# ndjinga/CirculantPreconditioner

Measured on AMD Instinct MI355X. Metric: PCApply/s on 256^3 complex grid, higher is better.
Workload: dtype c128 (f64 complex); 1 GPU; 256x256x256 c128 circulant PCApply, transport symbol lambda=(0.6, 0.15, 0.02); global_batch=1, parallelism=single GPU

## Files before the change

circulantpreconditioner_amd/csrc/cfp_three_pass.hip:

```cpp
#include "cfp_fft_device.h"
#include "cfp_lane.h"
#include "cfp_three_pass.h"

#include <hip/hip_ext.h>

#ifndef CFP_REAL_MID_XCD
#define CFP_REAL_MID_XCD 1
#endif

#define TP_LAUNCH(K, G, B, S, ...)                                                                    \
  do {                                                                                                \
    if (g_stamp.start || g_stamp.stop)                                                                \
      hipExtLaunchKernelGGL(K, G, B, 0, S, g_stamp.start, g_stamp.stop, 0, __VA_ARGS__);              \
    else                                                                                              \
      hipLaunchKernelGGL(K, G, B, 0, S, __VA_ARGS__);                                                 \
  } while (0)

namespace cfp {

namespace {

__device__ __forceinline__ cd dft4_dif(cd v, int q) {
  const cd p = dpp_c<DPP_XOR2>(v);
  cd t = (q & 2) ? csub(p, v) : cadd(v, p);
// ... 411 lines not shown
    }
    {
      const Col q = column(u);
#pragma unroll
      for (int m = 0; m < PTS; ++m)
        if constexpr (!(PROBE & PR_NO_Y2)) v[m] = dft4_dit(v[m], q.y2 & 3);
#pragma unroll
      for (int m = 0; m < PTS; ++m) {
        if constexpr ((PROBE & PR_NO_Y2) != 0) {
          v[m] = cmul(v[m], q.w);
          continue;
        }
        if constexpr (N2 >= 8) {
          const cd u = (q.y2 & 4) ? cmul(v[m], q.w8) : v[m];
          const cd p = lane_xor4(u);
          v[m] = (q.y2 & 4) ? csub(p, u) : cadd(u, p);
        }
        if constexpr (N2 == 16) {
          const cd u = (q.y2 & 8) ? cmul(v[m], q.w16) : v[m];
          const cd p = lane_xor8(u);
          v[m] = (q.y2 & 8) ? csub(p, u) : cadd(u, p);
        }
        v[m] = cmul(v[m], q.w);
      }
      if constexpr (PROBE & PR_NO_STORE) {
        double acc = 0.0;
#pragma unroll
        for (int m = 0; m < PTS; ++m) acc += v[m].x + v[m].y;
        if (acc == 1.2345e300) q.col[0] = make_cd(acc, 0.0);
      } else {
#pragma unroll
        for (int m = 0; m < PTS; ++m) gstore<FLAGS>(q.col + zs * TZ * m, cconj(v[m]));
      }
    }
    lds_barrier();
  }
}

namespace {
__device__ __forceinline__ double ror8_d(double v) {
  const long long b = __double_as_longlong(v);
  const int lo = __builtin_amdgcn_mov_dpp((int)(b & 0xffffffffll), 0x128, 0xf, 0xf, false);
  const int hi = __builtin_amdgcn_mov_dpp((int)(b >> 32), 0x128, 0xf, 0xf, false);
  return __longlong_as_double(((long long)hi << 32) | (unsigned int)lo);
}
__device__ __forceinline__ cd bfly_l3(cd v, double sgn) {
  return make_cd(fma(sgn, v.x, ror8_d(v.x)), fma(sgn, v.y, ror8_d(v.y)));
}
}

template <int B, int D, bool TW = true, int NR = 16>
__device__ __forceinline__ void dif_pairs(cd* v, cd w) {
#pragma unroll
  for (int k = 0; k < NR; ++k)
    if ((k & D) == 0) swap_c<B>(v[k], v[k + D]);
#pragma unroll
  for (int k = 0; k < NR; ++k)
    if ((k & D) == 0) {
      const cd a = v[k], b = v[k + D];
      v[k] = cadd(a, b);
      v[k + D] = TW ? cmul(csub(a, b), w) : csub(a, b);
    }
}

typedef __attribute__((address_space(3))) void lds_void_t;
typedef __attribute__((address_space(1))) void glb_void_t;
template <int T, int N2, int TN, int PROBE = 0, bool PF = false, int NX = TN, int ST = 0, int LD = 0, bool BL = false,
          bool XCD = false, int TAG = 0>
__global__ void __launch_bounds__(T * (TN / 16)) __attribute__((amdgpu_waves_per_eu(4)))
k_tp_mid_sw(cd* data, TPArgs a, int nunits) {
#ifndef CFP_KEXP
  static_assert(PROBE == 0, "timing probes are built in tools/kexp only");
#endif
  static_assert(T == 64 || (T == 32 && N2 == 8), "a wave = the 64 columns of one z group, or 32 columns of two");
  static_assert(N2 == 4 || N2 == 8, "y2 = the top 2 or 3 lane bits");
  static_assert(TN == 256, "z = 16 x 16: radix-16 stage A in registers, one exchange, radix-16 stage B");
  constexpr int N1 = TN / N2, TZ = TN / 16, NT = T * TZ, XT = T / N2, NXT = NX / XT;
  constexpr int XB = ilog2(XT);
  static_assert(NX % XT == 0, "whole x tiles");
  static_assert(!BL || (NX == TN && N2 == 8), "blocked layout: complex grid, 8 x times 8 y2");
  __shared__ __attribute__((aligned(16))) double lds[T * TN];
  __shared__ cd tw_l[TN];
  const int tid = threadIdx.x;
  for (int i = tid; i < TN; i += NT) tw_l[i] = a.tw[i];
  __syncthreads();
  const int lane0 = tid & 63;
  const int c0 = T == 64 ? lane0 : (lane0 & 3) | ((lane0 >> 3) << 2);
  const int tz0 = T == 64 ? tid / 64 : 2 * (tid >> 6) + ((lane0 >> 2) & 1);
  const i64 zs = (i64)NX << (a.lnyl ? a.lnyl : ilog2(TN));
  const auto idx = [](int i) {
    asm volatile("" : "+v"(i));
    return i;
  };
  const auto col_ptr = [&](int u, int c, int tz) {
    const int xt = u % NXT, k1 = u / NXT;
    if constexpr (BL) return data + (i64)NX * N2 * k1 + xt * T + c + zs * tz;
    return data + xt * XT + (c & (XT - 1)) + (i64)NX * ((c >> XB) + N2 * k1) + zs * tz;
  };
  const auto tw_y = [&](int u, int c) { return tw_l[((c >> XB) * (a.k1_off + u / NXT)) & (TN - 1)]; };
  constexpr int NPF = PF ? 8 : 0;
  const int wv = __builtin_amdgcn_readfirstlane(tid / 64);
  if constexpr ((PROBE & PR_PRIO) != 0) {
    if (wv >= NT / 128) __builtin_amdgcn_s_setprio(1);
  }
  const auto prefetch = [&](int u) {
    const int c = idx(c0), tz = idx(tz0);
    const cd* src = col_ptr(u, c, tz);
#pragma unroll
    for (int m = 0; m < NPF; ++m)
      __builtin_amdgcn_global_load_lds((glb_void_t*)(src + zs * TZ * m), (lds_void_t*)(lds + (wv * NPF + m) * 128),
                                       16, 0, (LD & F_NT_LD) ? 2 : 0);
  };
  static_assert(!PF || (NT / 64) * NPF * 128 <= T * TN, "the prefetch fits the exchange buffer");
  if constexpr (PF) {
    if ((int)blockIdx.x < nunits) prefetch(XCD ? xcd_unit(blockIdx.x, gridDim.x) : (int)blockIdx.x);
  }
  const auto exchange_t = [&](cd* v, bool first) {
    if constexpr (PROBE & PR_NO_XCHG) return;
    const int c = idx(c0), tz = idx(tz0), lane = idx(lane0);
    const int l3 = N2 == 8 ? ((lane >> 3) & 1) : 0, l4 = (lane >> 4) & 1, l5 = (lane >> 5) & 1;
    const int wbase = (tz * 16 + l5 + 2 * l4) * T + (c & (XT - 1)) + XT * l3;
#pragma unroll
    for (int h = 0; h < 2; ++h) {
      if (!(first && h == 0)) lds_barrier();
#pragma unroll
      for (int r = 0; r < 16; ++r) {
        const int p = N2 == 8 ? 4 * (r & 1) + 2 * ((r >> 1) & 1) : 2 * (r & 1) + ((r >> 1) & 1);
        const int off = (r & 12) * T + XT * (N2 == 8 ? p & 6 : p);
        lds[wbase + off] = h ? v[r].y : v[r].x;
      }
      lds_barrier();
#pragma unroll
      for (int t = 0; t < 16; ++t) {
        const double d = lds[(tz + TZ * t) * T + c];
        if (h) v[t].y = d; else v[t].x = d;
      }
    }
  };
  const auto stage_b = [&](cd* v) {
    if constexpr (PROBE & PR_NO_ZMATH) return;
    const int tz = idx(tz0);
#pragma unroll
    for (int t = 1; t < 16; ++t) v[t] = cmul(v[t], tw_l[tz * t]);
    dft_reg<16>(v);
  };
  const auto lane_sign = [&]() {
    const int lane = idx(lane0);
    return (lane & 8) ? -1.0 : 1.0;
  };

  for (int it = blockIdx.x; it < nunits; it += gridDim.x) {
    const int u = XCD ? xcd_unit(it, gridDim.x) : it;
    cd v[16];
    if constexpr (PROBE & PR_NO_LOAD) {
      const int c = idx(c0), tz = idx(tz0);
#pragma unroll
      for (int m = 0; m < 16; ++m) v[m] = make_cd(c + m, tz + u);
    } else {
      const int c = idx(c0), tz = idx(tz0);
      const cd* src = col_ptr(u, c, tz);
#pragma unroll
      for (int m = NPF; m < 16; ++m) v[m] = gload<LD>(src + zs * TZ * m);
      if constexpr (PF) {
        asm volatile("s_waitcnt vmcnt(0)" ::: "memory");
#pragma unroll
        for (int m = 0; m < NPF; ++m) {
          const int lane = idx(lane0);
          v[m] = fromv(*reinterpret_cast<const dv2*>(lds + (wv * NPF + m) * 128 + 2 * lane));
        }
      }
    }
    {
      const int c = idx(c0);
      const cd w = tw_y(u, c);
#pragma unroll
      for (int m = 0; m < 16; ++m) v[m] = cmul(v[m], w);
    }
    if constexpr (!(PROBE & PR_NO_ZMATH)) dft_reg<16>(v);
    if constexpr (PROBE & PR_NO_Y2) {
    } else if constexpr (N2 == 8) {
      {
        const int lane = idx(lane0);
        dif_pairs<5, 1>(v, tw_l[(TN / 8) * ((lane >> 3) & 3)]);
      }
      {
        const int lane = idx(lane0);
        dif_pairs<4, 2>(v, tw_l[(TN / 4) * ((lane >> 3) & 1)]);
      }
      const double s = lane_sign();
#pragma unroll
      for (int r = 0; r < 16; ++r) v[r] = bfly_l3(v[r], s);
    } else {
      {
        const int lane = idx(lane0);
        dif_pairs<5, 1>(v, tw_l[(TN / 4) * ((lane >> 4) & 1)]);
      }
      dif_pairs<4, 2, false>(v, make_cd(1.0, 0.0));
    }
    exchange_t(v, !PF);
    stage_b(v);
    {
      const int c = idx(c0), tz = idx(tz0);
      const int k1 = a.k1_off + u / NXT, p = c >> XB;
      const cd cs = a.colsym[(u % NXT) * XT + (c & (XT - 1)) + (i64)NX * (k1 + N1 * brev<N2>(p))];
#pragma unroll
      for (int m = 0; m < 16; ++m) {
        const cd d = cadd(cadd(cs, a.axsym[tz + TZ * m]), make_cd(1.0, 0.0));
        v[m] = (PROBE & PR_NO_ZMATH) ? cconj(v[m]) : cconj(cdiv_sym(v[m], d));
      }
    }
    if constexpr (!(PROBE & PR_NO_ZMATH)) dft_reg<16>(v);
    if constexpr (PROBE & PR_NO_Y2) {
    } else if constexpr (N2 == 8) {
      {
        const double s = lane_sign();
#pragma unroll
        for (int r = 0; r < 16; ++r) v[r] = bfly_l3(v[r], s);
      }
      {
        const int lane = idx(lane0);
        const cd w = tw_l[(TN / 4) * ((lane >> 3) & 1)];
#pragma unroll
        for (int k = 0; k < 16; ++k)
          if ((k & 2) == 0) swap_c<4>(v[k], v[k + 2]);
#pragma unroll
        for (int k = 0; k < 16; ++k)
          if ((k & 2) == 0) {
            const cd x = v[k], y = cmul(v[k + 2], w);
            v[k] = cadd(x, y);
            v[k + 2] = csub(x, y);
          }
      }
      {
        const int lane = idx(lane0);
        const cd w = tw_l[(TN / 8) * ((lane >> 3) & 1)];
#pragma unroll
        for (int k = 0; k < 16; ++k)
          if ((k & 1) == 0) swap_c<5>(v[k], v[k + 1]);
#pragma unroll
        for (int k = 0; k < 16; ++k)
          if ((k & 1) == 0) {
            cd y = cmul(v[k + 1], w);
            if (k & 2) y = mul_mi(y);
            const cd x = v[k];
            v[k] = cadd(x, y);
            v[k + 1] = csub(x, y);
          }
      }
    } else {
#pragma unroll
      for (int k = 0; k < 16; ++k)
        if ((k & 2) == 0) swap_c<4>(v[k], v[k + 2]);
#pragma unroll
      for (int k = 0; k < 16; ++k)
        if ((k & 2) == 0) {
          const cd x = v[k], y = v[k + 2];
          v[k] = cadd(x, y);
          v[k + 2] = csub(x, y);
        }
#pragma unroll
      for (int k = 0; k < 16; ++k)
        if ((k & 1) == 0) swap_c<5>(v[k], v[k + 1]);
#pragma unroll
      for (int k = 0; k < 16; ++k)
        if ((k & 1) == 0) {
          const cd y = (k & 2) ? mul_mi(v[k + 1]) : v[k + 1];
          const cd x = v[k];
          v[k] = cadd(x, y);
          v[k + 1] = csub(x, y);
        }
    }
    exchange_t(v, false);
    if constexpr (PF) {
      lds_barrier();
      if (it + (int)gridDim.x < nunits) prefetch(XCD ? xcd_unit(it + gridDim.x, gridDim.x) : it + (int)gridDim.x);
    }
    stage_b(v);
    {
      const int c = idx(c0), tz = idx(tz0);
      const cd w = tw_y(u, c);
      cd* dst = col_ptr(u, c, tz);
      if constexpr (PROBE & PR_NO_STORE) {
        double acc = 0.0;
#pragma unroll
        for (int m = 0; m < 16; ++m) acc += v[m].x * w.x + v[m].y;
        if (acc == 1.2345e300) dst[0] = make_cd(acc, 0.0);
      } else {
#pragma unroll
        for (int m = 0; m < 16; ++m) gstore<ST>(dst + zs * TZ * m, cconj(cmul(v[m], w)));
      }
    }
    if constexpr (!PF) lds_barrier();
  }
}

constexpr int kRecNPF = 7;
template <int PROBE, bool PF, int LD>
__device__ __forceinline__ void tp_mid_rec_body(cd* __restrict__ data, const TPArgs& a, int nunits,
                                                double* __restrict__ pf_l, cd* __restrict__ carr,
                                                cd* __restrict__ ctab, cd* __restrict__ tw_l) {
  constexpr int TN = 256, N2 = 8, N1 = TN / N2, XT = 8, NXT = TN / XT, NW = 16;
  constexpr int NPF = PF ? kRecNPF : 0;
  const int tid = threadIdx.x;
  const int lane = tid & 63, x = lane & 7, zl = lane >> 3;
  const int wv = __builtin_amdgcn_readfirstlane(tid / 64);
  const i64 zs = (i64)TN << (a.lnyl ? a.lnyl : ilog2(TN));
  const cd lz = a.lamz;
  const auto idx = [](int i) {
    asm volatile("" : "+v"(i));
    return i;
  };
  const auto colsym_of = [&](int u) {
    return a.colsym[(u % NXT) * XT + x + (i64)TN * (a.k1_off + u / NXT + N1 * zl)];
  };
  const auto ctab_put = [&](int buf, cd cs) {
    const cd den = make_cd(cs.x + 1.0 + lz.x, cs.y + lz.y);
    const double id = 1.0 / fma(den.x, den.x, den.y * den.y);
    const cd ri = make_cd(den.x * id, -den.y * id);
    ctab[(2 * buf) * 64 + idx(lane)] = cmul(lz, ri);
    ctab[(2 * buf + 1) * 64 + idx(lane)] = make_cd(ri.x * (double)TN, ri.y * (double)TN);
  };
  if (tid < TN) tw_l[tid] = a.tw[tid];
  if (wv == 0 && (int)blockIdx.x < nunits) ctab_put(0, colsym_of((int)blockIdx.x));
  __syncthreads();
  const unsigned loff = 16u * ((unsigned)x + (unsigned)zs * 2u * (unsigned)zl);
  const auto slot_ptr = [&](int u, int m) {
    return data + ((u % NXT) * XT + (i64)TN * (N2 * (u / NXT) + (m & 7)) + zs * (16 * wv + (m >> 3)));
  };
  const auto at = [](cd* base, unsigned off) { return reinterpret_cast<cd*>(reinterpret_cast<char*>(base) + off); };
  const auto prefetch = [&](int u) {
    unsigned lo0 = loff;
    asm volatile("" : "+s"(u), "+v"(lo0));
#pragma unroll
    for (int m = 0; m < NPF; ++m)
      __builtin_amdgcn_global_load_lds((glb_void_t*)at(slot_ptr(u, m), lo0), (lds_void_t*)(pf_l + (wv * NPF + m) * 128),
                                       16, 0, (LD & F_NT_LD) ? 2 : 0);
  };
  if constexpr (PF) {
    if ((int)blockIdx.x < nunits) prefetch((int)blockIdx.x);
  }
  const bool up3 = (zl & 1) != 0, up4 = (zl & 2) != 0, up5 = (zl & 4) != 0;
  const cd zero = make_cd(0.0, 0.0), one = make_cd(1.0, 0.0);
  const auto pin = [](cd& w) { asm volatile("" : "+v"(w.x), "+v"(w.y)); };
  const auto cfma = [](cd p, cd q, cd c) {
    return make_cd(fma(p.x, q.x, fma(-p.y, q.y, c.x)), fma(p.x, q.y, fma(p.y, q.x, c.y)));
  };

  int par = 0, buf = 0;
  const auto unit = [&](const int it, auto more_c) {
    constexpr bool more = decltype(more_c)::value;
    const int u = it;
    const int k1 = a.k1_off + u / NXT;
    const int nbuf = buf == 2 ? 0 : buf + 1;
    cd v[16], csn = zero;
    if constexpr (PROBE & PR_NO_LOAD) {
#pragma unroll
      for (int m = 0; m < 16; ++m) v[m] = make_cd(lane + m, wv + u);
    } else {
      if constexpr (PF) {
        asm volatile("s_waitcnt vmcnt(0)" ::: "memory");
#pragma unroll
        for (int m = 0; m < NPF; ++m)
          v[m] = fromv(*reinterpret_cast<const dv2*>(pf_l + (wv * NPF + m) * 128 + 2 * idx(lane)));
      }
      if constexpr (more) csn = colsym_of(it + (int)gridDim.x);
      {
        int ul = u;
        unsigned lo1 = loff;
        asm volatile("" : "+s"(ul), "+v"(lo1));
#pragma unroll
        for (int m = NPF; m < 16; ++m) v[m] = gload<LD>(at(slot_ptr(ul, m), lo1));
      }
    }
    if (more && wv == 0) ctab_put(nbuf, csn);
#pragma unroll
    for (int y = 1; y < N2; ++y) {
      const cd w = tw_l[(y * k1) & (TN - 1)];
      v[y] = cmul(v[y], w);
      v[8 + y] = cmul(v[8 + y], w);
    }
    if constexpr (PF && more && !(PROBE & PR_NO_LOAD)) {
#pragma unroll
      for (int m = 0; m < 16; ++m) pin(v[m]);
      prefetch(it + (int)gridDim.x);
    }
    __builtin_amdgcn_sched_barrier(0);
    if constexpr (!(PROBE & PR_NO_Y2)) {
      dft_reg<8>(v);
#pragma unroll
      for (int m = 0; m < 8; ++m) pin(v[m]);
      __builtin_amdgcn_sched_barrier(0);
      dft_reg<8>(v + 8);
#pragma unroll
      for (int m = 8; m < 16; ++m) pin(v[m]);
      __builtin_amdgcn_sched_barrier(0);
    }
    if constexpr (!(PROBE & PR_NO_ZMATH)) {
      const auto pow2zl = [&](cd aa) {
        cd pw = cmul(aa, aa), q = up3 ? pw : one;
        pw = cmul(pw, pw);
        q = up4 ? cmul(q, pw) : q;
        pw = cmul(pw, pw);
        return up5 ? cmul(q, pw) : q;
      };
#pragma unroll
      for (int k2 = 0; k2 < 8; ++k2) {
        const int c = (idx(lane) & 7) + 8 * k2;
        const cd aa = ctab[(2 * buf) * 64 + c], r = ctab[(2 * buf + 1) * 64 + c];
        const cd v0 = cmul(v[k2], r), v1 = cmul(v[8 + k2], r);
        cd S = cfma(aa, v0, v1), X, lo, hi, pw = cmul(aa, aa), q;
        __builtin_amdgcn_sched_barrier(0);
        {
          const cd pr = lane_xor8(S);
          lo = up3 ? pr : S;
          hi = up3 ? S : pr;
          X = up3 ? lo : zero;
          S = cfma(pw, lo, hi);
          q = up3 ? pw : one;
          pw = cmul(pw, pw);
        }
        __builtin_amdgcn_sched_barrier(0);
        {
          lo = S;
          hi = S;
          swap_c<4>(lo, hi);
          if (up4) X = cfma(q, lo, X);
          S = cfma(pw, lo, hi);
          q = up4 ? cmul(q, pw) : q;
          pw = cmul(pw, pw);
        }
        __builtin_amdgcn_sched_barrier(0);
        {
          lo = S;
          hi = S;
          swap_c<5>(lo, hi);
          if (up5) X = cfma(q, lo, X);
          S = cfma(pw, lo, hi);
        }
        v[k2] = cfma(aa, X, v0);
        v[8 + k2] = cfma(aa, v[k2], v1);
        pin(v[k2]);
        pin(v[8 + k2]);
        if (zl == k2) carr[(par * NW + wv) * 64 + idx(lane)] = S;
        __builtin_amdgcn_sched_barrier(0);
      }
      lds_barrier();
      cd cin;
      {
        const int ln = idx(lane);
        const cd am = ctab[(2 * buf) * 64 + ln];
        const cd am2 = cmul(am, am), am4 = cmul(am2, am2), am8 = cmul(am4, am4);
        const cd A = cmul(am8, am8);
        cd acc = carr[(par * NW + wv) * 64 + ln];
#pragma unroll
        for (int k = 14; k >= 0; --k) {
          acc = cfma(acc, A, carr[(par * NW + ((wv - 1 - k) & 15)) * 64 + ln]);
          if ((k & 3) == 0) __builtin_amdgcn_sched_barrier(0);
        }
        const cd A2 = cmul(A, A), A4 = cmul(A2, A2), A8 = cmul(A4, A4), A16 = cmul(A8, A8);
        const cd d = make_cd(1.0 - A16.x, -A16.y);
        const double id = 1.0 / fma(d.x, d.x, d.y * d.y);
        cin = make_cd(fma(acc.x, d.x, acc.y * d.y) * id, fma(acc.y, d.x, -acc.x * d.y) * id);
      }
#pragma unroll
      for (int k2 = 0; k2 < 8; ++k2) {
        const int c = (idx(lane) & 7) + 8 * k2;
        const long long bx = __double_as_longlong(cin.x), by = __double_as_longlong(cin.y);
        const unsigned xl = (unsigned)__builtin_amdgcn_ds_bpermute(4 * c, (int)(bx & 0xffffffffll));
        const unsigned xh = (unsigned)__builtin_amdgcn_ds_bpermute(4 * c, (int)(bx >> 32));
        const unsigned yl = (unsigned)__builtin_amdgcn_ds_bpermute(4 * c, (int)(by & 0xffffffffll));
        const unsigned yh = (unsigned)__builtin_amdgcn_ds_bpermute(4 * c, (int)(by >> 32));
        const cd ci = make_cd(__longlong_as_double((long long)(((unsigned long long)xh << 32) | xl)),
                              __longlong_as_double((long long)(((unsigned long long)yh << 32) | yl)));
        const cd aa = ctab[(2 * buf) * 64 + c];
        const cd g = cmul(cmul(aa, pow2zl(aa)), ci);
        v[k2] = cadd(v[k2], g);
        v[8 + k2] = cfma(aa, g, v[8 + k2]);
        pin(v[k2]);
        pin(v[8 + k2]);
        __builtin_amdgcn_sched_barrier(0);
      }
    }
#pragma unroll
    for (int m = 0; m < 16; ++m) v[m] = cconj(v[m]);
    if constexpr (!(PROBE & PR_NO_Y2)) {
      dft_reg<8>(v);
#pragma unroll
      for (int m = 0; m < 8; ++m) pin(v[m]);
      __builtin_amdgcn_sched_barrier(0);
      dft_reg<8>(v + 8);
#pragma unroll
      for (int m = 8; m < 16; ++m) pin(v[m]);
      __builtin_amdgcn_sched_barrier(0);
    }
    {
      int k1s = k1, us = u;
      unsigned lo2 = loff;
      asm volatile("" : "+s"(k1s), "+s"(us), "+v"(lo2));
      if constexpr (PROBE & PR_NO_STORE) {
        double acc = 0.0;
#pragma unroll
        for (int m = 0; m < 16; ++m) acc += v[m].x + v[m].y;
        if (acc == 1.2345e300) *at(slot_ptr(us, 0), lo2) = make_cd(acc, 0.0);
      } else {
#pragma unroll
        for (int m = 0; m < 16; ++m) {
          const cd w = (m & 7) ? tw_l[((m & 7) * k1s) & (TN - 1)] : one;
          gstore<0>(at(slot_ptr(us, m), lo2), cconj(cmul(v[m], w)));
        }
      }
    }
    par ^= 1;
    buf = nbuf;
  };
  int it = blockIdx.x;
  for (; it + (int)gridDim.x < nunits; it += gridDim.x) unit(it, std::true_type{});
  if (it < nunits) unit(it, std::false_type{});
}

template <int PROBE = 0, bool PF = false, int LD = 0, int TAG = 0>
__global__ void __launch_bounds__(1024) __attribute__((amdgpu_waves_per_eu(4)))
k_tp_mid_rec(cd* data, TPArgs a, int nunits) {
#ifndef CFP_KEXP
  static_assert(PROBE == 0, "timing probes are built in tools/kexp only");
#endif
  __shared__ __attribute__((aligned(16))) double pf_l[PF ? 16 * kRecNPF * 128 : 2];
  __shared__ __attribute__((aligned(16))) cd carr[2 * 16 * 64];
  __shared__ __attribute__((aligned(16))) cd ctab[3 * 2 * 64];
  __shared__ cd tw_l[256];
  tp_mid_rec_body<PROBE, PF, LD>(data, a, nunits, pf_l, carr, ctab, tw_l);
}


bool three_pass_supported(const i64 n[3]) {
  return n[0] == n[1] && n[1] == n[2] && (n[0] == 128 || n[0] == 256 || n[0] == 512);
}

static int cu_count() {
  static int cus = 0;
  if (!cus) {
    int dev = 0;
    if (hipGetDevice(&dev) != hipSuccess ||
        hipDeviceGetAttribute(&cus, hipDeviceAttributeMultiprocessorCount, dev) != hipSuccess || cus < 1)
      cus = 256;
  }
  return cus;
}

static unsigned grid_of(int units, int per_cu) {
  const int g = per_cu * cu_count();
  return (unsigned)(units < g ? units : g);
}
static unsigned grid_xcd(int units, int per_cu) {
  unsigned g = grid_of(units, per_cu), p = 1;
  while (2 * p <= g) p *= 2;
  return p >= 8 && units % p == 0 ? p : 0;
}

template <bool INV, int M = 128, int N1 = 32, int N2 = 8, int NY = 256, int MF = 0, int OCC = 4, bool WC = false,
          bool WL = false>
__global__ void __launch_bounds__(N1 * (M / 8)) __attribute__((amdgpu_waves_per_eu(OCC)))
k_tp_rows_r2c(const double* in_r, cd* H, cd* Q, double* out_r, TPArgs a, int nunits) {
  constexpr int PTS = 8;
  constexpr int TPC = M / PTS;
  constexpr int TY = N1 / PTS;
  constexpr int NT = N1 * TPC;
  constexpr int RS = M + M / 16;
  constexpr int TC = WL ? M + 16 : M;
  static_assert(!WL || (64 % TPC == 0 && TY * 16 == 64 && M % 16 == 0), "wave-local: whole rows and 16 columns per wave");
  constexpr int F = (WC ? 0 : F_SPLIT_LDS) | F_LDS_SYNC;
  constexpr int FW = F | (WL ? F_WAVE_LDS : 0);
  constexpr int LDS_D = (N1 * RS > N1 * TC ? N1 * RS : N1 * TC) * (WC ? 2 : 1);
  __shared__ __attribute__((aligned(16))) double lds[LDS_D];
  cd* const lc = reinterpret_cast<cd*>(lds);
  __shared__ cd tw_m[M];
  __shared__ cd tw_1[N1];
  __shared__ cd qy[N1];
  const int tid = threadIdx.x;
  for (int i = tid; i < M; i += NT) tw_m[i] = a.tw[2 * i];
  for (int i = tid; i < N1; i += NT) tw_1[i] = a.tw[(2 * M / N1) * i];
  if constexpr (WL) __syncthreads();
  const int r0 = tid / TPC, tpc0 = tid % TPC;
  const int x0 = WL ? (tid >> 6) * 16 + (tid & 15) : tid % M, ty0 = WL ? (tid >> 4) & 3 : tid / M;
  const auto idx = [](int i) {
    asm volatile("" : "+v"(i));
    return i;
  };
  const auto to_columns_r2c = [&](cd* v, int z, int y2) {
    const int r = idx(r0), tpc = idx(tpc0), x = idx(x0), ty = idx(ty0);
    const int xm = (M - x) & (M - 1);
    cd zm[PTS];
    if constexpr (WC) {
      lds_barrier();
#pragma unroll
      for (int t = 0; t < PTS; ++t) {
        const int k = tpc + TPC * t;
        lc[r * RS + k + (k >> 4)] = v[t];
      }
      lds_barrier();
#pragma unroll
      for (int m = 0; m < PTS; ++m) {
        const int row = (ty + TY * m) * RS;
        v[m] = lc[row + x + (x >> 4)];
        zm[m] = lc[row + xm + (xm >> 4)];
      }
    } else {
#pragma unroll
      for (int h = 0; h < 2; ++h) {
        lds_barrier();
#pragma unroll
        for (int t = 0; t < PTS; ++t) {
          const int k = tpc + TPC * t;
          lds[r * RS + k + (k >> 4)] = h ? v[t].y : v[t].x;
        }
        lds_barrier();
#pragma unroll
        for (int m = 0; m < PTS; ++m) {
          const int row = (ty + TY * m) * RS;
          const double d = lds[row + x + (x >> 4)], dm = lds[row + xm + (xm >> 4)];
          if (h) { v[m].y = d; zm[m].y = dm; } else { v[m].x = d; zm[m].x = dm; }
        }
      }
    }
    lds_barrier();
    const cd w = a.tw[x];
#pragma unroll
    for (int m = 0; m < PTS; ++m) {
      const cd e = make_cd(0.5 * (v[m].x + zm[m].x), 0.5 * (v[m].y - zm[m].y));
      const cd d = make_cd(v[m].x - zm[m].x, v[m].y + zm[m].y);
      const cd o = make_cd(0.5 * d.y, -0.5 * d.x);
      v[m] = cadd(e, cmul(w, o));
      if (x == 0) qy[ty + TY * m] = csub(e, o);
    }
  };
  const auto to_rows_c2r = [&](cd* v, int z, int y2) {
    const int r = idx(r0), tpc = idx(tpc0), x = idx(x0), ty = idx(ty0);
    cd xm[PTS];
    if constexpr (WC) {
      lds_barrier();
#pragma unroll
      for (int m = 0; m < PTS; ++m) lc[(ty + TY * m) * RS + x + (x >> 4)] = cconj(v[m]);
      lds_barrier();
#pragma unroll
      for (int t = 0; t < PTS; ++t) {
        const int k = tpc + TPC * t, km = (M - k) & (M - 1);
        v[t] = lc[r * RS + k + (k >> 4)];
        xm[t] = lc[r * RS + km + (km >> 4)];
      }
    } else {
#pragma unroll
      for (int h = 0; h < 2; ++h) {
        lds_barrier();
#pragma unroll
        for (int m = 0; m < PTS; ++m) lds[(ty + TY * m) * RS + x + (x >> 4)] = h ? -v[m].y : v[m].x;
        lds_barrier();
#pragma unroll
        for (int t = 0; t < PTS; ++t) {
          const int k = tpc + TPC * t, km = (M - k) & (M - 1);
          const double d = lds[r * RS + k + (k >> 4)], dm = lds[r * RS + km + (km >> 4)];
          if (h) { v[t].y = d; xm[t].y = dm; } else { v[t].x = d; xm[t].x = dm; }
        }
      }
    }
    lds_barrier();
    if (tpc == 0) xm[0] = qy[r];
#pragma unroll
    for (int t = 0; t < PTS; ++t) {
      const int k = tpc + TPC * t;
      const cd e = make_cd(0.5 * (v[t].x + xm[t].x), 0.5 * (v[t].y - xm[t].y));
      const cd d = make_cd(0.5 * (v[t].x - xm[t].x), 0.5 * (v[t].y + xm[t].y));
      const cd o = cmul(d, cconj(a.tw[k]));
      v[t] = cconj(make_cd(e.x - o.y, e.y + o.x));
    }
  };
  for (int u = blockIdx.x; u < nunits; u += gridDim.x) {
    const int z = u / N2, y2 = u % N2;
    cd v[PTS];
    if constexpr (!INV) {
      {
        const int r = idx(r0), tpc = idx(tpc0);
        const cd* src = reinterpret_cast<const cd*>(in_r) + ((i64)z * NY + y2 + N2 * r) * M + tpc;
#pragma unroll
        for (int t = 0; t < PTS; ++t) v[t] = gload<MF>(src + TPC * t);
        __builtin_amdgcn_sched_barrier(0);
        fft_stages<M, PTS, r0_of(M, PTS), true, N1, FW>(v, lds, tw_m, r, tpc, true);
      }
      to_columns_r2c(v, z, y2);
      {
        const int x = idx(x0), ty = idx(ty0);
        fft_stages<N1, PTS, r0_of(N1, PTS), false, TC, FW>(v, lds, tw_1, x, ty, true);
        cd* dst = H + ((i64)z * NY + y2 + N2 * ty) * M + x;
#pragma unroll
        for (int m = 0; m < PTS; ++m) dst[(i64)N2 * TY * M * m] = v[m];
      }
      if constexpr (WL) asm volatile("s_waitcnt lgkmcnt(0)" ::: "memory");
      if (tid < N1) {
        const int k = idx(tid);
        cd acc = make_cd(0.0, 0.0);
#pragma unroll 8
        for (int j = 0; j < N1; ++j) acc = cadd(acc, cmul(qy[j], tw_1[(j * k) & (N1 - 1)]));
        Q[(i64)z * NY + y2 + N2 * k] = acc;
      }
    } else {
      cd qk = make_cd(0.0, 0.0);
      if (tid < N1) qk = Q[(i64)z * NY + y2 + N2 * idx(tid)];
      {
        const int x = idx(x0), ty = idx(ty0);
        const cd* src = H + ((i64)z * NY + y2 + N2 * ty) * M + x;
#pragma unroll
        for (int m = 0; m < PTS; ++m) v[m] = src[(i64)N2 * TY * M * m];
        __builtin_amdgcn_sched_barrier(0);
#pragma unroll
        for (int m = 0; m < PTS; ++m) v[m] = cconj(v[m]);
        fft_stages<N1, PTS, r0_of(N1, PTS), false, TC, FW>(v, lds, tw_1, x, ty, true);
      }
      if (tid < 64) {
        if (tid < N1) qy[tid] = qk;
        asm volatile("s_waitcnt lgkmcnt(0)" ::: "memory");
        cd acc = make_cd(0.0, 0.0);
        const int y1 = idx(tid) & (N1 - 1);
#pragma unroll 8
        for (int k = 0; k < N1; ++k) acc = cadd(acc, cmul(qy[k], cconj(tw_1[(y1 * k) & (N1 - 1)])));
        asm volatile("s_waitcnt lgkmcnt(0)" ::: "memory");
        if (tid < N1) qy[tid] = acc;
      }
      to_rows_c2r(v, z, y2);
      {
        const int r = idx(r0), tpc = idx(tpc0);
        fft_stages<M, PTS, r0_of(M, PTS), true, N1, FW>(v, lds, tw_m, r, tpc, true);
        const double sc = a.scale;
        cd* dst = reinterpret_cast<cd*>(out_r) + ((i64)z * NY + y2 + N2 * r) * M + tpc;
#pragma unroll
        for (int t = 0; t < PTS; ++t) gstore<MF>(dst + TPC * t, make_cd(v[t].x * sc, -v[t].y * sc));
      }
    }
    lds_barrier();
  }
}

hipError_t launch_three_pass_real(int stage, int n, const double* b, cd* H, cd* Q, double* x, const TPArgs& a,
                                  hipStream_t s, bool alt_rows) {
  if (stage == 3) {
    if (n == 128)
      hipLaunchKernelGGL((k_tp_mid<0, 4, 4, 128, 8, false, 1>), dim3(32), dim3(4 * 16), 0, s, Q, a, 32);
    else
      hipLaunchKernelGGL((k_tp_mid<0, 8, 8, 256, 4, false, 1>), dim3(32), dim3(8 * 64), 0, s, Q, a, 32);
    return hipGetLastError();
  }
  if (n == 128) {
    if (stage == 1) {
      constexpr int units = (64 / 8) * 32;
      hipLaunchKernelGGL((k_tp_mid<0, 32, 4, 128, 8, false, 64>), dim3(grid_of(units, 2)), dim3(512), 0, s, H, a,
                         units);
    } else {
      constexpr int units = 128 * 4;
      const unsigned g = grid_of(units, 4);
      if (stage == 0 && alt_rows)
        hipLaunchKernelGGL((k_tp_rows_r2c<false, 64, 32, 4, 128>), dim3(g), dim3(256), 0, s, b, H, Q, nullptr, a,
                           units);
      else if (stage == 0)
        hipLaunchKernelGGL((k_tp_rows_r2c<false, 64, 32, 4, 128, 0, 4, false, true>), dim3(g), dim3(256), 0, s, b, H,
                           Q, nullptr, a, units);
      else if (alt_rows)
        hipLaunchKernelGGL((k_tp_rows_r2c<true, 64, 32, 4, 128>), dim3(g), dim3(256), 0, s, nullptr, H, Q, x, a,
                           units);
      else
        hipLaunchKernelGGL((k_tp_rows_r2c<true, 64, 32, 4, 128, 0, 4, false, true>), dim3(g), dim3(256), 0, s, nullptr,
                           H, Q, x, a, units);
    }
    return hipGetLastError();
  }
  if (stage == 1) {
    constexpr int units = (128 / 8) * 32;
    const unsigned gx = CFP_REAL_MID_XCD ? grid_xcd(units, 1) : 0;
    if (gx)
      hipLaunchKernelGGL((k_tp_mid_sw<64, 8, 256, 0, true, 128, 0, 0, false, true>), dim3(gx), dim3(1024), 0, s, H, a,
                         units);
    else
      hipLaunchKernelGGL((k_tp_mid_sw<64, 8, 256, 0, true, 128>), dim3(grid_of(units, 1)), dim3(1024), 0, s, H, a,
                         units);
  } else {
    constexpr int units = 256 * 8;
    const unsigned g = grid_of(units, 2);
    if (stage == 0 && !alt_rows)
      hipLaunchKernelGGL((k_tp_rows_r2c<false, 128, 32, 8, 256, F_NT_LD, 6, false, true>), dim3(grid_of(units, 3)),
                         dim3(512), 0, s, b, H, Q, nullptr, a, units);
    else if (stage == 0)
      hipLaunchKernelGGL((k_tp_rows_r2c<false, 128, 32, 8, 256, F_NT_LD, 6>), dim3(grid_of(units, 3)), dim3(512), 0, s, b,
                         H, Q, nullptr, a, units);
    else if (!alt_rows)
      hipLaunchKernelGGL((k_tp_rows_r2c<true, 128, 32, 8, 256, F_NT_ST, 4, true, true>), dim3(g), dim3(512), 0, s,
                         nullptr, H, Q, x, a, units);
    else
      hipLaunchKernelGGL((k_tp_rows_r2c<true, 128, 32, 8, 256, F_NT_ST, 4, true>), dim3(g), dim3(512), 0, s, nullptr, H, Q, x, a,
                         units);
  }
  return hipGetLastError();
}


constexpr int kP1Flags = F_NT_LD, kP1InPlaceFlags = 0;
constexpr int kP3Flags = F_NT_ST;
constexpr bool kRowsLP = true;
constexpr int kP2LoadFlags = F_NT_LD;
constexpr bool kRowsWave = true;
constexpr bool kRowsXCD = CFP_ROWS_XCD != 0;

template <int N1, int TN, int PER_CU, int PTS = 16, bool XS = true, bool LP = false, int BL = 0, bool XCD = false,
          int P1F = kP1Flags, int P3F = kP3Flags, bool WR = kRowsWave>
static void launch_rows(int stage, const cd* in, cd* out, const TPArgs& a, hipStream_t s) {
  constexpr int units = TN * (TN / N1);
  constexpr int W = WR ? F_WAVE_LDS : 0;
// ... 265 lines not shown
```

Measured before the change: 3593 PCApply/s.

## Transpose mid-pass lane mapping: y-DFT across lanes, z recurrence in registers

```diff
diff --git a/circulantpreconditioner_amd/csrc/cfp_three_pass.hip b/circulantpreconditioner_amd/csrc/cfp_three_pass.hip
--- a/circulantpreconditioner_amd/csrc/cfp_three_pass.hip
+++ b/circulantpreconditioner_amd/csrc/cfp_three_pass.hip
@@ -737,7 +737,7 @@
   constexpr int TN = 256, N2 = 8, N1 = TN / N2, XT = 8, NXT = TN / XT, NW = 16;
   constexpr int NPF = PF ? kRecNPF : 0;
   const int tid = threadIdx.x;
-  const int lane = tid & 63, x = lane & 7, zl = lane >> 3;
+  const int lane = tid & 63, x = lane & 7, y2 = lane >> 3;
   const int wv = __builtin_amdgcn_readfirstlane(tid / 64);
   const i64 zs = (i64)TN << (a.lnyl ? a.lnyl : ilog2(TN));
   const cd lz = a.lamz;
@@ -746,7 +746,7 @@
     return i;
   };
   const auto colsym_of = [&](int u) {
-    return a.colsym[(u % NXT) * XT + x + (i64)TN * (a.k1_off + u / NXT + N1 * zl)];
+    return a.colsym[(u % NXT) * XT + x + (i64)TN * (a.k1_off + u / NXT + N1 * brev<N2>(y2))];
   };
   const auto ctab_put = [&](int buf, cd cs) {
     const cd den = make_cd(cs.x + 1.0 + lz.x, cs.y + lz.y);
@@ -758,9 +758,9 @@
   if (tid < TN) tw_l[tid] = a.tw[tid];
   if (wv == 0 && (int)blockIdx.x < nunits) ctab_put(0, colsym_of((int)blockIdx.x));
   __syncthreads();
-  const unsigned loff = 16u * ((unsigned)x + (unsigned)zs * 2u * (unsigned)zl);
+  const unsigned loff = 16u * ((unsigned)x + (unsigned)TN * (unsigned)y2);
   const auto slot_ptr = [&](int u, int m) {
-    return data + ((u % NXT) * XT + (i64)TN * (N2 * (u / NXT) + (m & 7)) + zs * (16 * wv + (m >> 3)));
+    return data + ((u % NXT) * XT + (i64)TN * N2 * (u / NXT) + zs * (16 * wv + m));
   };
   const auto at = [](cd* base, unsigned off) { return reinterpret_cast<cd*>(reinterpret_cast<char*>(base) + off); };
   const auto prefetch = [&](int u) {
@@ -774,8 +774,27 @@
   if constexpr (PF) {
     if ((int)blockIdx.x < nunits) prefetch((int)blockIdx.x);
   }
-  const bool up3 = (zl & 1) != 0, up4 = (zl & 2) != 0, up5 = (zl & 4) != 0;
-  const cd zero = make_cd(0.0, 0.0), one = make_cd(1.0, 0.0);
+  const cd zero = make_cd(0.0, 0.0);
+  const double s3 = (y2 & 1) ? -1.0 : 1.0;
+  const cd w8 = a.tw[(TN / 8) * (y2 & 3)], w4 = a.tw[(TN / 4) * (y2 & 1)];
+  const auto dif2 = [](auto bit, cd& p, cd& q, cd w) {
+    constexpr int B = decltype(bit)::value;
+    swap_c<B>(p, q);
+    const cd s = cadd(p, q), d = cmul(csub(p, q), w);
+    p = s;
+    q = d;
+    swap_c<B>(p, q);
+  };
+  const auto dit2 = [](auto bit, cd& p, cd& q, cd w) {
+    constexpr int B = decltype(bit)::value;
+    swap_c<B>(p, q);
+    const cd t = cmul(q, w);
+    q = csub(p, t);
+    p = cadd(p, t);
+    swap_c<B>(p, q);
+  };
+  using bit5 = std::integral_constant<int, 5>;
+  using bit4 = std::integral_constant<int, 4>;
   const auto pin = [](cd& w) { asm volatile("" : "+v"(w.x), "+v"(w.y)); };
   const auto cfma = [](cd p, cd q, cd c) {
     return make_cd(fma(p.x, q.x, fma(-p.y, q.y, c.x)), fma(p.x, q.y, fma(p.y, q.x, c.y)));
@@ -808,85 +827,39 @@
       }
     }
     if (more && wv == 0) ctab_put(nbuf, csn);
-#pragma unroll
-    for (int y = 1; y < N2; ++y) {
-      const cd w = tw_l[(y * k1) & (TN - 1)];
-      v[y] = cmul(v[y], w);
-      v[8 + y] = cmul(v[8 + y], w);
-    }
-    if constexpr (PF && more && !(PROBE & PR_NO_LOAD)) {
-#pragma unroll
-      for (int m = 0; m < 16; ++m) pin(v[m]);
-      prefetch(it + (int)gridDim.x);
+    {
+      const cd w = tw_l[((idx(lane) >> 3) * k1) & (TN - 1)];
+#pragma unroll
+      for (int m = 0; m < 16; ++m) v[m] = cmul(v[m], w);
     }
     __builtin_amdgcn_sched_barrier(0);
     if constexpr (!(PROBE & PR_NO_Y2)) {
-      dft_reg<8>(v);
-#pragma unroll
-      for (int m = 0; m < 8; ++m) pin(v[m]);
-      __builtin_amdgcn_sched_barrier(0);
-      dft_reg<8>(v + 8);
-#pragma unroll
-      for (int m = 8; m < 16; ++m) pin(v[m]);
-      __builtin_amdgcn_sched_barrier(0);
+#pragma unroll
+      for (int m = 0; m < 16; m += 2) {
+        dif2(bit5{}, v[m], v[m + 1], w8);
+        dif2(bit4{}, v[m], v[m + 1], w4);
+        v[m] = bfly_l3(v[m], s3);
+        v[m + 1] = bfly_l3(v[m + 1], s3);
+        pin(v[m]);
+        pin(v[m + 1]);
+        if ((m & 2) == 2) __builtin_amdgcn_sched_barrier(0);
+      }
     }
     if constexpr (!(PROBE & PR_NO_ZMATH)) {
-      const auto pow2zl = [&](cd aa) {
-        cd pw = cmul(aa, aa), q = up3 ? pw : one;
-        pw = cmul(pw, pw);
-        q = up4 ? cmul(q, pw) : q;
-        pw = cmul(pw, pw);
-        return up5 ? cmul(q, pw) : q;
-      };
-#pragma unroll
-      for (int k2 = 0; k2 < 8; ++k2) {
-        const int c = (idx(lane) & 7) + 8 * k2;
-        const cd aa = ctab[(2 * buf) * 64 + c], r = ctab[(2 * buf + 1) * 64 + c];
-        const cd v0 = cmul(v[k2], r), v1 = cmul(v[8 + k2], r);
-        cd S = cfma(aa, v0, v1), X, lo, hi, pw = cmul(aa, aa), q;
-        __builtin_amdgcn_sched_barrier(0);
-        {
-          const cd pr = lane_xor8(S);
-          lo = up3 ? pr : S;
-          hi = up3 ? S : pr;
-          X = up3 ? lo : zero;
-          S = cfma(pw, lo, hi);
-          q = up3 ? pw : one;
-          pw = cmul(pw, pw);
-        }
-        __builtin_amdgcn_sched_barrier(0);
-        {
-          lo = S;
-          hi = S;
-          swap_c<4>(lo, hi);
-          if (up4) X = cfma(q, lo, X);
-          S = cfma(pw, lo, hi);
-          q = up4 ? cmul(q, pw) : q;
-          pw = cmul(pw, pw);
-        }
-        __builtin_amdgcn_sched_barrier(0);
-        {
-          lo = S;
-          hi = S;
-          swap_c<5>(lo, hi);
-          if (up5) X = cfma(q, lo, X);
-          S = cfma(pw, lo, hi);
-        }
-        v[k2] = cfma(aa, X, v0);
-        v[8 + k2] = cfma(aa, v[k2], v1);
-        pin(v[k2]);
-        pin(v[8 + k2]);
-        if (zl == k2) carr[(par * NW + wv) * 64 + idx(lane)] = S;
-        __builtin_amdgcn_sched_barrier(0);
-      }
+      const int ln = idx(lane);
+      const cd aa = ctab[(2 * buf) * 64 + ln];
+#pragma unroll
+      for (int m = 1; m < 16; ++m) v[m] = cfma(aa, v[m - 1], v[m]);
+      const cd E = cmul(ctab[(2 * buf + 1) * 64 + ln], v[15]);
+      carr[(par * NW + wv) * 64 + ln] = E;
+#pragma unroll
+      for (int m = 0; m < 16; ++m) pin(v[m]);
       lds_barrier();
       cd cin;
       {
-        const int ln = idx(lane);
-        const cd am = ctab[(2 * buf) * 64 + ln];
-        const cd am2 = cmul(am, am), am4 = cmul(am2, am2), am8 = cmul(am4, am4);
+        const cd am2 = cmul(aa, aa), am4 = cmul(am2, am2), am8 = cmul(am4, am4);
         const cd A = cmul(am8, am8);
-        cd acc = carr[(par * NW + wv) * 64 + ln];
+        cd acc = E;
 #pragma unroll
         for (int k = 14; k >= 0; --k) {
           acc = cfma(acc, A, carr[(par * NW + ((wv - 1 - k) & 15)) * 64 + ln]);
@@ -897,52 +870,47 @@
         const double id = 1.0 / fma(d.x, d.x, d.y * d.y);
         cin = make_cd(fma(acc.x, d.x, acc.y * d.y) * id, fma(acc.y, d.x, -acc.x * d.y) * id);
       }
-#pragma unroll
-      for (int k2 = 0; k2 < 8; ++k2) {
-        const int c = (idx(lane) & 7) + 8 * k2;
-        const long long bx = __double_as_longlong(cin.x), by = __double_as_longlong(cin.y);
-        const unsigned xl = (unsigned)__builtin_amdgcn_ds_bpermute(4 * c, (int)(bx & 0xffffffffll));
-        const unsigned xh = (unsigned)__builtin_amdgcn_ds_bpermute(4 * c, (int)(bx >> 32));
-        const unsigned yl = (unsigned)__builtin_amdgcn_ds_bpermute(4 * c, (int)(by & 0xffffffffll));
-        const unsigned yh = (unsigned)__builtin_amdgcn_ds_bpermute(4 * c, (int)(by >> 32));
-        const cd ci = make_cd(__longlong_as_double((long long)(((unsigned long long)xh << 32) | xl)),
-                              __longlong_as_double((long long)(((unsigned long long)yh << 32) | yl)));
-        const cd aa = ctab[(2 * buf) * 64 + c];
-        const cd g = cmul(cmul(aa, pow2zl(aa)), ci);
-        v[k2] = cadd(v[k2], g);
-        v[8 + k2] = cfma(aa, g, v[8 + k2]);
-        pin(v[k2]);
-        pin(v[8 + k2]);
-        __builtin_amdgcn_sched_barrier(0);
-      }
-    }
-#pragma unroll
-    for (int m = 0; m < 16; ++m) v[m] = cconj(v[m]);
-    if constexpr (!(PROBE & PR_NO_Y2)) {
-      dft_reg<8>(v);
-#pragma unroll
-      for (int m = 0; m < 8; ++m) pin(v[m]);
-      __builtin_amdgcn_sched_barrier(0);
-      dft_reg<8>(v + 8);
-#pragma unroll
-      for (int m = 8; m < 16; ++m) pin(v[m]);
-      __builtin_amdgcn_sched_barrier(0);
+      const cd r = ctab[(2 * buf + 1) * 64 + ln];
+      cd g = cmul(aa, cin);
+#pragma unroll
+      for (int m = 0; m < 16; ++m) {
+        v[m] = cfma(r, v[m], g);
+        if (m < 15) g = cmul(aa, g);
+      }
     }
     {
       int k1s = k1, us = u;
       unsigned lo2 = loff;
       asm volatile("" : "+s"(k1s), "+s"(us), "+v"(lo2));
+      const cd w = tw_l[((idx(lane) >> 3) * k1s) & (TN - 1)];
+#pragma unroll
+      for (int m = 0; m < 16; m += 2) {
+        cd p = cconj(v[m]), q = cconj(v[m + 1]);
+        if constexpr (!(PROBE & PR_NO_Y2)) {
+          p = bfly_l3(p, s3);
+          q = bfly_l3(q, s3);
+          dit2(bit4{}, p, q, w4);
+          dit2(bit5{}, p, q, w8);
+        }
+        v[m] = cconj(cmul(p, w));
+        v[m + 1] = cconj(cmul(q, w));
+        pin(v[m]);
+        pin(v[m + 1]);
+        if ((m & 2) == 2) __builtin_amdgcn_sched_barrier(0);
+      }
+      if constexpr (PF && more && !(PROBE & PR_NO_LOAD)) {
+        prefetch(it + (int)gridDim.x);
+        __builtin_amdgcn_sched_barrier(0);
+      }
+      if constexpr (!(PROBE & PR_NO_STORE)) {
+#pragma unroll
+        for (int m = 0; m < 16; ++m) gstore<0>(at(slot_ptr(us, m), lo2), v[m]);
+      }
       if constexpr (PROBE & PR_NO_STORE) {
         double acc = 0.0;
 #pragma unroll
         for (int m = 0; m < 16; ++m) acc += v[m].x + v[m].y;
         if (acc == 1.2345e300) *at(slot_ptr(us, 0), lo2) = make_cd(acc, 0.0);
-      } else {
-#pragma unroll
-        for (int m = 0; m < 16; ++m) {
-          const cd w = (m & 7) ? tw_l[((m & 7) * k1s) & (TN - 1)] : one;
-          gstore<0>(at(slot_ptr(us, m), lo2), cconj(cmul(v[m], w)));
-        }
       }
     }
     par ^= 1;
```

New measurement: 3731 PCApply/s, median of 6. 1.04x the previous value.
